# MasonMcGill/multipath-nn

Measured on AMD Instinct MI355X. Metric: images/sec training CIFAR-10 actor-net, higher is better.
Workload: dtype f32; 1 GPU; cifar10-ac: ac_chain(k_cpt=0) 8-block actor-routed chain, 32x32x3, 10 classes; global_batch=128, per_gpu_batch=128, parallelism=dp1, rccl_ranks=1, hip_graph=True, steps_per_graph=4, streams=1, clock_warmup_steps=96

## Files before the change

### multipath-nn_amd/csrc/lin.hip

```cpp
#include "common.h"
#include <cstddef>

struct LinFwdG {
    ActG a;  int HW;
    gptr<const float> w[2];  gptr<const float> b[2];  gptr<float> y[2];  int M[2];
    gptr<const float> k_cpt;  float alpha_cpt;  int extra_col[2];
    int n;
    gptr<float> kpart;  gptr<int> kcnt;
};
struct LinBwdG {
    ActG a;  int HW;
    gptr<const float> w[2];  gptr<const float> dy[2];  int M[2];
    gptr<float> dw[2];  gptr<float> db[2];
    gptr<float> dx;
    gptr<const float> k_cpt;  float alpha_cpt;  int extra_col[2];
    int n;
    gptr<float> dz_out;  gptr<double> red_out;  int red_nslot;
    gptr<float> kpart;  gptr<int> kcnt;
    float act_alpha;  gptr<const float> act_w;
};
static_assert(sizeof(LinFwdG) == sizeof(mpnn_lin_fwd_args) && offsetof(LinFwdG, y) == offsetof(mpnn_lin_fwd_args, y) &&
              offsetof(LinFwdG, k_cpt) == offsetof(mpnn_lin_fwd_args, k_cpt) && offsetof(LinFwdG, kcnt) == offsetof(mpnn_lin_fwd_args, kcnt),
              "LinFwdG mirrors mpnn_lin_fwd_args");
static_assert(sizeof(LinBwdG) == sizeof(mpnn_lin_bwd_args) && offsetof(LinBwdG, dw) == offsetof(mpnn_lin_bwd_args, dw) &&
// ... 280 lines not shown
#pragma unroll
            for (int s = 0; s < 8; ++s)
#pragma unroll
                for (int pp = 0; pp < LB_GP; ++pp) dx[pp] = __builtin_amdgcn_mfma_f32_16x16x4f32(ady[pp][s], wv[s], dx[pp], 0, 0, 0);
#pragma unroll
            for (int pp = 0; pp < LB_GP; ++pp)
#pragma unroll
                for (int s = 0; s < 4; ++s) {
                    accW[0] = __builtin_amdgcn_mfma_f32_16x16x4f32(xa[pp][s], bdy[pp][0][s], accW[0], 0, 0, 0);
                    accW[1] = __builtin_amdgcn_mfma_f32_16x16x4f32(xa[pp][s], bdy[pp][1][s], accW[1], 0, 0, 0);
                }
            asm volatile("" : "+a"(accW[0]), "+a"(accW[1]));
            mfma_drain();
            if (act_on) {
                const float a2 = 2.f * a.act_alpha;
#pragma unroll
                for (int pp = 0; pp < LB_GP; ++pp)
#pragma unroll
                    for (int q = 0; q < 4; ++q) {
                        const int rr = LB_ROWS * (pg + pp) + 4 * g + q;
                        const bool ok = rr < nr && f < K;
                        const float w = a.act_w[ok ? R0 + rr : R0];
                        dx[pp][q] += ok ? a2 * w * xa[pp][q] : 0.f;
                    }
            }
#pragma unroll
            for (int pp = 0; pp < LB_GP; ++pp)
#pragma unroll
                for (int q = 0; q < 4; ++q) {
                    const int rr = LB_ROWS * (pg + pp) + 4 * g + q;
                    if (rr < nr && f < K) {
                        if (a.dx) a.dx[(size_t)(R0 + rr) * K + f] = dx[pp][q];
                        if (fuse_bn) {
                            const float dz = xa[pp][q] > 0.f ? dx[pp][q] : 0.f;
                            a.dz_out[(size_t)(R0 + rr) * K + f] = dz;
                            r1 += dz; r2 += dz * xh[pp][q];
                        }
                    }
                }
        }
    }
    trace_stamp(4);
    float dbt = 0.f;
    if (blockIdx.x == 0) {
        float *dbp = tr + 512;
        dbp[tid] = dbs;
        __syncthreads();
        if (tid < 32) {
#pragma unroll
            for (int rg = 0; rg < 8; ++rg) dbt += dbp[rg * 32 + tid];
        }
    }
    if constexpr (RS) {
        if (Z > 1) {
            __shared__ int ticket;
            const gptr<float> part0 = a.kpart + (size_t)blockIdx.x * gridDim.z * MPNN_LIN_RS_TILE;
            const gptr<float> mine = part0 + (size_t)zi * MPNN_LIN_RS_TILE;
#pragma unroll
            for (int set = 0; set < 2; ++set)
#pragma unroll
                for (int q = 0; q < 4; ++q)
                    __hip_atomic_store(mine + (wid * 16 + 4 * g + q) * 32 + set * 16 + li, accW[set][q], __ATOMIC_RELAXED, __HIP_MEMORY_SCOPE_SYSTEM);
            if (blockIdx.x == 0 && tid < 32) __hip_atomic_store(mine + 2048 + tid, dbt, __ATOMIC_RELAXED, __HIP_MEMORY_SCOPE_SYSTEM);
            asm volatile("s_waitcnt vmcnt(0)" ::: "memory");
            __builtin_amdgcn_fence(__ATOMIC_RELEASE, "workgroup");
            __syncthreads();
            if (tid == 0) ticket = __hip_atomic_fetch_add(a.kcnt + blockIdx.x, 1, __ATOMIC_RELAXED, __HIP_MEMORY_SCOPE_SYSTEM);
            __syncthreads();
            if (ticket != Z - 1) { trace_stamp(5); goto bn_sums; }
            {
                float pv[2][4][MPNN_LIN_RSPLIT];
#pragma unroll
                for (int set = 0; set < 2; ++set)
#pragma unroll
                    for (int q = 0; q < 4; ++q)
#pragma unroll
                        for (int z = 0; z < MPNN_LIN_RSPLIT; ++z)
                            pv[set][q][z] = __hip_atomic_load(part0 + (size_t)(z < Z ? z : 0) * MPNN_LIN_RS_TILE + (wid * 16 + 4 * g + q) * 32 + set * 16 + li,
                                                              __ATOMIC_RELAXED, __HIP_MEMORY_SCOPE_SYSTEM);
                float pd[MPNN_LIN_RSPLIT];
#pragma unroll
                for (int z = 0; z < MPNN_LIN_RSPLIT; ++z)
                    pd[z] = (blockIdx.x == 0 && tid < 32) ? __hip_atomic_load(part0 + (size_t)(z < Z ? z : 0) * MPNN_LIN_RS_TILE + 2048 + tid, __ATOMIC_RELAXED, __HIP_MEMORY_SCOPE_SYSTEM) : 0.f;
#pragma unroll
                for (int set = 0; set < 2; ++set)
#pragma unroll
                    for (int q = 0; q < 4; ++q) {
                        float v = 0.f;
#pragma unroll
                        for (int z = 0; z < MPNN_LIN_RSPLIT; ++z) v += z < Z ? pv[set][q][z] : 0.f;
                        accW[set][q] = v;
                    }
                dbt = 0.f;
#pragma unroll
                for (int z = 0; z < MPNN_LIN_RSPLIT; ++z) dbt += z < Z ? pd[z] : 0.f;
                if (tid == 0) __hip_atomic_store(a.kcnt + blockIdx.x, 0, __ATOMIC_RELAXED, __HIP_MEMORY_SCOPE_SYSTEM);
            }
        }
    }
#pragma unroll
    for (int set = 0; set < 2; ++set) {
        const gptr<const float> wp = set ? a.w[1] : a.w[0];
        const gptr<float> dwp = set ? a.dw[1] : a.dw[0];
        if (!wp || !dwp) continue;
        const int M = set ? a.M[1] : a.M[0];
        const int krows = (set ? a.extra_col[1] : a.extra_col[0]) ? K + 1 : K;
// ... 57 lines not shown
```

### multipath-nn_amd/csrc/route.hip

```cpp
#include "common.h"

#define MSK MPNN_MAX_SINKS

#define RT_THREADS 512
#define RT_WAVES (RT_THREADS / 64)

__device__ __forceinline__ int4 uniform4(int4 v) {
    return make_int4(__builtin_amdgcn_readfirstlane(v.x), __builtin_amdgcn_readfirstlane(v.y),
                     __builtin_amdgcn_readfirstlane(v.z), __builtin_amdgcn_readfirstlane(v.w));
}

template <class P, class T> __device__ __forceinline__ void st_part(P p, T v) { __hip_atomic_store(p, v, __ATOMIC_RELAXED, __HIP_MEMORY_SCOPE_SYSTEM); }
template <class P> __device__ __forceinline__ auto ld_part(P p) { return __hip_atomic_load(p, __ATOMIC_RELAXED, __HIP_MEMORY_SCOPE_SYSTEM); }

struct RouteG {
    int net_type;  int n_nodes, n_leaves, n_switches, max_sinks;
    int optimistic, use_cls_err, want_grad;
    gptr<const int> nodes;  gptr<const int> sw_children;  gptr<const float> node_ops;
    gptr<const float> hyp;
    gptr<const float> k_cpt_vec;
    gptr<const float> r;
    gptr<const float> c_err;  gptr<const float> d_cor;
    gptr<float> p_tr, p_ev;
    gptr<float> w_cerr;
    gptr<float> dr;
    gptr<float> node_stat;
    gptr<double> loss;
    int n;  int n_total;
    gptr<float> stat_part;  gptr<int> stat_ticket;
};
static_assert(sizeof(RouteG) == sizeof(mpnn_route_args) && offsetof(RouteG, nodes) == offsetof(mpnn_route_args, nodes) &&
              offsetof(RouteG, loss) == offsetof(mpnn_route_args, loss) && offsetof(RouteG, n_total) == offsetof(mpnn_route_args, n_total) &&
              offsetof(RouteG, stat_ticket) == offsetof(mpnn_route_args, stat_ticket), "RouteG mirrors mpnn_route_args");

template <int RB, class A>
__device__ __forceinline__ void route_body(const A &a, const int blk, const int nblk) {
    extern __shared__ __attribute__((aligned(16))) float lds[];
    const int n = a.n, NN = a.n_nodes, MS = a.max_sinks;
    const bool det_stat = a.node_stat && a.stat_part && nblk > 2;
    trace_stamp(0); trace_note(6, 14);
    float *P = lds;
    float *PE = P + NN * RB;
    float *V = PE + NN * RB;
    float *O = V + NN * RB;
    float *RIN = O + NN * RB;
    float *CE = RIN + a.n_switches * MS * RB;
    float *DC = CE + a.n_leaves * RB;
    float *SM = DC + a.n_leaves * RB;
    int *ARG = (int *)(SM + a.n_switches * MS * RB);
    int4 *REC = (int4 *)(ARG + a.n_switches * RB);
    float *OPS = (float *)(REC + NN + 1);
    int *SWN = (int *)(OPS + NN);
    const int s0 = blk * RB;
// ... 247 lines not shown
    if (a.loss) {
        const double e = wave_sum_d(live ? (double)l_err : 0.0), c = wave_sum_d(live ? (double)l_cpt : 0.0);
        const double x = wave_sum_d(live ? (double)l_aux : 0.0), cnt = wave_sum_d((live && wave == 0) ? 1.0 : 0.0);
        double *lsum = (double *)lds;
        __syncthreads();
        if (lane_t == 0) { lsum[wave * 4] = e; lsum[wave * 4 + 1] = c; lsum[wave * 4 + 2] = x; lsum[wave * 4 + 3] = wave == 0 ? cnt : 0.0; }
        __syncthreads();
        if (threadIdx.x < 4) {
            double t = 0.0;
#pragma unroll
            for (int w = 0; w < RT_WAVES; ++w) t += lsum[w * 4 + threadIdx.x];
            if (det_stat) st_part(pcast<double>(a.stat_part + (size_t)nblk * NN * 2) + blk * 4 + threadIdx.x, t);
            else atomic_add_g(a.loss + threadIdx.x, t);
        }
    }
    if (det_stat) {
        int *last_s = (int *)lds + 128;
        asm volatile("s_waitcnt vmcnt(0)" ::: "memory");
        __syncthreads();
        if (threadIdx.x == 0) {
            __threadfence();
            *last_s = atomic_add_g(a.stat_ticket, 1) == nblk - 1;
        }
        __syncthreads();
        if (*last_s) {
            __threadfence();
            for (int i = threadIdx.x; i < 2 * NN; i += RT_THREADS) {
                float t = 0.f;
                for (int b = 0; b < nblk; ++b) t += ld_part(a.stat_part + (size_t)b * NN * 2 + i);
                a.node_stat[i] += t;
            }
            if (a.loss && threadIdx.x < 4) {
                const auto lp = pcast<const double>(a.stat_part + (size_t)nblk * NN * 2);
                double t = 0.0;
                for (int b = 0; b < nblk; ++b) t += ld_part(lp + b * 4 + threadIdx.x);
                a.loss[threadIdx.x] += t;
            }
            if (threadIdx.x == 0) *a.stat_ticket = 0;
        }
    }
    trace_stamp(5);
}

template <int RB>
__global__ __launch_bounds__(RT_THREADS) void route_k(const mpnn_route_args a) { route_body<RB>(a, blockIdx.x, gridDim.x); }

template <int RB>
__global__ __launch_bounds__(RT_THREADS) void route_multi_k(const mpnn_route_args *__restrict__ tab, const int wpn) {
    const int net = blockIdx.x / wpn;
    const RouteG a = ((const RouteG *)tab)[net];
    route_body<RB>(a, blockIdx.x - net * wpn, wpn);
}

int mpnn_trace_install_route(void *buf) { return mpnn_trace_install(buf); }

extern "C" int mpnn_route(const mpnn_route_args *args, void *stream) {
    if (!args || !args->nodes || !args->p_tr || !args->p_ev || (args->stat_part && !args->stat_ticket)) return MPNN_E_ARG;
    if (args->n_nodes > MPNN_MAX_NODES || args->max_sinks > MPNN_MAX_SINKS) return MPNN_E_SHAPE;
    if (args->n <= 0) return 0;
    const size_t per = (size_t)(4 * args->n_nodes + 2 * args->n_switches * args->max_sinks + args->n_switches + 2 * args->n_leaves) * 4;
    const size_t fix = (size_t)(args->n_nodes * 5 + 8 + args->n_switches) * 4;
    const size_t cap = 160 * 1024;
    const hipStream_t st = (hipStream_t)stream;
    const int n = args->n;
    static bool raised = false;
    if (!raised) {
        hipFuncSetAttribute((const void *)route_k<64>, hipFuncAttributeMaxDynamicSharedMemorySize, (int)cap);
        hipFuncSetAttribute((const void *)route_k<32>, hipFuncAttributeMaxDynamicSharedMemorySize, (int)cap);
        hipFuncSetAttribute((const void *)route_k<16>, hipFuncAttributeMaxDynamicSharedMemorySize, (int)cap);
        raised = true;
    }
    if (per * 64 + fix <= cap)      hipLaunchKernelGGL(route_k<64>, dim3((n + 63) / 64), dim3(RT_THREADS), per * 64 + fix, st, *args);
    else if (per * 32 + fix <= cap) hipLaunchKernelGGL(route_k<32>, dim3((n + 31) / 32), dim3(RT_THREADS), per * 32 + fix, st, *args);
    else if (per * 16 + fix <= cap) hipLaunchKernelGGL(route_k<16>, dim3((n + 15) / 16), dim3(RT_THREADS), per * 16 + fix, st, *args);
    else return MPNN_E_SHAPE;
    MPNN_LAUNCH_CHECK();
    return 0;
}

extern "C" int mpnn_route_multi(const mpnn_route_args *host_table, const mpnn_route_args *dev_table, int count, void *stream) {
    if (count <= 0) return 0;
    if (!host_table || !dev_table) return MPNN_E_ARG;
    const mpnn_route_args *args = host_table;
    for (int k = 0; k < count; ++k) {
        const mpnn_route_args &b = host_table[k];
        if (!b.nodes || !b.p_tr || !b.p_ev || (b.stat_part && !b.stat_ticket)) return MPNN_E_ARG;
        if (b.n != args->n || b.n_nodes != args->n_nodes || b.n_switches != args->n_switches || b.n_leaves != args->n_leaves ||
            b.max_sinks != args->max_sinks) return MPNN_E_ARG;
    }
    if (args->n_nodes > MPNN_MAX_NODES || args->max_sinks > MPNN_MAX_SINKS) return MPNN_E_SHAPE;
    if (args->n <= 0) return 0;
    const size_t per = (size_t)(4 * args->n_nodes + 2 * args->n_switches * args->max_sinks + args->n_switches + 2 * args->n_leaves) * 4;
    const size_t fix = (size_t)(args->n_nodes * 5 + 8 + args->n_switches) * 4;
    const size_t cap = 160 * 1024;
    const hipStream_t st = (hipStream_t)stream;
    const int n = args->n;
    static bool raised = false;
    if (!raised) {
        hipFuncSetAttribute((const void *)route_multi_k<64>, hipFuncAttributeMaxDynamicSharedMemorySize, (int)cap);
        hipFuncSetAttribute((const void *)route_multi_k<32>, hipFuncAttributeMaxDynamicSharedMemorySize, (int)cap);
        hipFuncSetAttribute((const void *)route_multi_k<16>, hipFuncAttributeMaxDynamicSharedMemorySize, (int)cap);
        raised = true;
    }
    if (per * 64 + fix <= cap)      { const int w = (n + 63) / 64; hipLaunchKernelGGL(route_multi_k<64>, dim3(w * count), dim3(RT_THREADS), per * 64 + fix, st, dev_table, w); }
    else if (per * 32 + fix <= cap) { const int w = (n + 31) / 32; hipLaunchKernelGGL(route_multi_k<32>, dim3(w * count), dim3(RT_THREADS), per * 32 + fix, st, dev_table, w); }
    else if (per * 16 + fix <= cap) { const int w = (n + 15) / 16; hipLaunchKernelGGL(route_multi_k<16>, dim3(w * count), dim3(RT_THREADS), per * 16 + fix, st, dev_table, w); }
    else return MPNN_E_SHAPE;
    MPNN_LAUNCH_CHECK();
    return 0;
}
```

### multipath-nn_amd/lib/_eng_planner.py

```python
import ctypes as C
import functools
import os

import numpy as np
import torch

from lib import _hip
from lib._eng_common import Launch, _attr, head_activity, head_parts


class Planner:

    def _wsplit(self, b, i, n, fused=False):
        H = b.H[i]
        tiles = n * (H // 16) * (H // 4) if H >= 16 else (n if H == 8 else (n + 3) // 4)
        nch = (b.Cin[i] + 15) // 16 + ((b.C[i - 1] + 15) // 16 if i > 0 else 0)
        groups = max(1, b.C[i] // 64) if b.C[i] % 64 == 0 else (b.C[i] // 32 if b.C[i] % 32 == 0 else b.C[i] // 16)
        if fused:
            groups = b.C[i] // 64 if b.C[i] % 64 == 0 else b.C[i] // 16
        budget = 512
        if fused:
            has_dgrad = 1 if (b.in_map is not None or i > 0) else 0
            dg_items = tiles * ((b.parent.C[b.in_map[i]] // 16 if b.parent is not None else 0) + (b.C[i - 1] // 16 if i > 0 else 0))
            slots = self.lib.mpnn_msconv_bwd_scale_slots(b.H[i], b.W[i], b.C[i], has_dgrad, 1 if i > 0 else 0, dg_items)
# ... 128 lines not shown
            return None
        used = sum(g * body[2] for g, body in zip(gx, bodies))
        while True:
            cand = [q for q in range(len(gx)) if gx[q] < bodies[q][3] and used + bodies[q][2] <= slots]
            if not cand:
                break
            q = max(cand, key=lambda q: -(-bodies[q][3] // gx[q]) * bodies[q][4])
            gx[q] += 1
            used += bodies[q][2]
        if os.environ.get('MPNN_PLAN_DEBUG'):
            print('level budget: %d slots, chain %.1f; ' % (slots, cands[lo]) + '; '.join(
                'm%d %s rows %d tiles %d -> gx %d (%d wgs, %d items/wg)' % (k, kind, rows, tiles, g, g * rows, -(-tiles // g))
                for (k, kind, rows, tiles, lat), g in zip(bodies, gx)))
        out = [dict(gxh=0, gxv=0, split=1) for _ in grp]
        for (k, kind, rows, tiles, lat), g in zip(bodies, gx):
            if self.co_share == 1:
                g = self._xcd_round(g)
            if kind == 'w':
                kb, b, i = grp[k]
                g = max(1, min(g, max(1, (12 << 20) // self._w_bytes(b, i))))
            out[k]['gxh' if kind == 'h' else 'gxv' if kind == 'v' else 'split'] = int(g)
        return out


    def program(self, mode, n, routed=False, gate=frozenset(), points=0):
        try:
            return self._program(mode, n, routed, frozenset(gate), int(points))
        finally:
            self.lib.mpnn_set_reserved_cus(0)


    def routed_prefix(self, n):
        table = self._ROUTED_PREFIX_GEN if self.generic_convs else self._ROUTED_PREFIX
        for lim, d0 in table:
            if n >= lim:
                return d0
        return table[-1][1]

    _ROUTED_PREFIX = ((6144, 1), (3072, 2), (1536, 3), (640, 4), (0, 6))
    _ROUTED_PREFIX_GEN = ((0, 1),)


    def _program(self, mode, n, routed, gate=frozenset(), points=0):
        if routed == 'auto':
            routed = n >= (self.routed_min_batch_gen if self.generic_convs else self.routed_min_batch)
        explicit = routed if (isinstance(routed, int) and not isinstance(routed, bool) and routed >= 1) else None
        routed = bool(routed) and mode != 'tr' and bool(self.switches) and self.net._net_kind != 'sr'
        if routed:
            routed = explicit if explicit is not None else self.routed_prefix(n)
        if mode == 'tr' and self.allreduce is not None and self.multi_stream:
            raise NotImplementedError('data-parallel training runs on the single-stream schedule (MPNN_STREAMS=0)')
        dp = mode == 'tr' and self.allreduce is not None
        reserve = self.dp_reserve_cus if (dp and len(self.dp_buckets) > 1) else 0
        key = (mode, n, self.multi_stream, self.group_fwd, routed, dp, self.bwd_levels, self.fold_clear, reserve, self.fuse_opt, self.co_share, gate) + \
            ((points,) if mode == 'ev+c' else ())
        if key in self._progs:
            return self._progs[key]
        self._ensure_capacity(n, mode == 'tr')
        if mode != 'tr':
            prog = self._progs[key] = self._program_ev(n, routed) if mode == 'ev' else self._program_cv(n, points) if mode == 'ev+c' else \
                self._program_pr(n, routed, mode == 'pr+p', gate)
            return prog
        if self.multi_stream and self.generic_convs:
            raise NotImplementedError('the multi-stream schedule has no launches for the general conv kernels (filters other '
                                      'than 3x3, maps other than the tuned squares): such nets run on the single-stream '
                                      'schedule (MPNN_STREAMS=0)')
        if self.multi_stream and any(len(b.children) > 1 for b in self.blocks):
            raise NotImplementedError('the multi-stream schedule serialises nothing between sibling blocks that '
                                      'accumulate into one gradient map: tree nets run on the single-stream schedule')
        prog = self._progs[key] = self._program_tr(n, dp, reserve)
        return prog


    def _program_tr(self, n, dp, reserve):
        sizes = sorted({h for b in self.blocks for h in b.H}, reverse=True)
        sid = {h: (0 if h == sizes[-1] else 1 + k) for k, h in enumerate(sizes)}
        self.n_streams = len(sizes) + 2
        fwd = self._label_map_launches(n) + self._lln_launches(n) + [Launch(None, 'fork')]
        if self.group_fwd and not self.multi_stream and self._groupable() and \
                all(b.parent is not None or b.in_map is None for b in self.blocks):
            for members in self._wavefront(self.blocks):
                fwd += self._conv_fwd_launches(members, n, 'tr')
        else:
            F = lambda b, i: 'F%d_%d' % (self.blocks.index(b), i)
            for b in self.blocks:
                for i in range(b.L):
                    fwd.append(self._conv_fwd_single(b, i, n, 'tr', None, 'msconv_fwd', stream=sid[b.H[i]],
                                                     waits=[F(b, i - 1)] if i > 0 else [], records=F(b, i)))
        fwd.append(Launch(None, 'join'))
        exit_fwd, bwd, fold = self._exit_launches(n)
        fwd += exit_fwd + [self._route_launch(n, 'tr', self.loss)]
        if dp and 'exit' in self.dp_buckets:
            bwd.append(Launch(None, 'bucket', tag='exit'))
        self.lib.mpnn_set_reserved_cus(reserve)
        convs, fused_opt = self._bwd_launches(n, sid, dp, reserve, fold)
        bwd += convs
        if dp:
            bwd.append(Launch(None, 'bucket', tag='end'))
        return dict(fwd=fwd, bwd=bwd, n=n, mode='tr', fold=fold, fused_opt=fused_opt)


    def _conv_fwd_args(self, b, i, n, mode, rows=None):
        train = mode == 'tr'
        a = _hip.ConvFwdArgs()
        a.a = self._act_of_input(b, i, n, _hip.ACT_BN_BATCH if train else _hip.ACT_BN_MOVING, fwd=train)
        cp = b.conv.params
        if i > 0:
            a.v, a.Cv = b.sp[i - 1].data_ptr(), b.C[i - 1]
            a.wv_pack = getattr(cp, 'w_vert_%i' % (i - 1)).data.data_ptr() if self.generic_convs else \
                self.packs[b.pack['w_vert_%i' % (i - 1)][0]:].data_ptr()
        if i < b.L - 1:
            a.pool_out = b.sp[i].data_ptr()
        a.wa_pack = getattr(cp, 'w_horz_%i' % i).data.data_ptr() if self.generic_convs else \
            self.packs[b.pack['w_horz_%i' % i][0]:].data_ptr()
        a.bias = getattr(b.conv.params, 'b_%i' % i).data.data_ptr()
        a.out = b.s[i].data_ptr()
        a.out_sum = self.dsum[b.sum_off[i]:].data_ptr() if train else None
        a.out_nslot = self._nslot(b, i)
        a.n, a.H, a.W, a.Cout = n, b.H[i], b.W[i], b.C[i]
        if rows is not None:
            a.idx, a.cnt = rows[0].data_ptr(), rows[1].data_ptr()
        return a


    @staticmethod
    def _conv_flops(b, i, n):
        (kh, kw), (kvh, kvw) = b.kh[i], b.kv[i] or (0, 0)
        return 2.0 * n * b.H[i] * b.W[i] * b.C[i] * (kh * kw * b.Cin[i] + (kvh * kvw * b.C[i - 1] if i > 0 else 0))


    def _conv_fwd_single(self, b, i, n, mode, rows, what, **kw):
        a = self._conv_fwd_args(b, i, n, mode, rows)
        self._keep.append(a)
        fl, tag = self._conv_flops(b, i, n), self._conv_tag(b, i)
        if self.generic_convs:
            return Launch(self._gen_fn('fwd'), what, C.byref(a), *b.kh[i], *(b.kv[i] or (0, 0)), flops=fl, tag=tag, **kw)
        return Launch(self.lib.mpnn_msconv_fwd, what, C.byref(a), flops=fl, tag=tag, **kw)


    @staticmethod
    def _conv_tag(b, i):
        hw = 'h%d' % b.H[i] if b.H[i] == b.W[i] else 'h%dx%d' % (b.H[i], b.W[i])
        return '%s %d+%d->%d' % (hw, b.Cin[i], b.C[i - 1] if i > 0 else 0, b.C[i])


    def _wavefront(self, blocks):
        depth = self._depths()
        kidx = {h: k for k, h in enumerate(sorted({h for b in self.blocks for h in b.H}, reverse=True))}
        levels = {}
        for b in blocks:
            for i in range(b.L):
                levels.setdefault(depth[id(b)] + kidx[b.H[i]], []).append((b, i))
        return [levels[d] for d in sorted(levels)]


    def _conv_fwd_launches(self, members, n, mode, rows=lambda b: None):
        lib, out = self.lib, []
        if not self._groupable():
            return [self._conv_fwd_single(b, i, n, mode, rows(b), 'fwd') for b, i in members]
        for c0 in range(0, len(members), 4):
            grp = members[c0:c0 + 4]
            arr = (_hip.ConvFwdArgs * len(grp))(*[self._conv_fwd_args(b, i, n, mode, rows(b)) for b, i in grp])
            dev_arr = _hip.to_device_table(list(arr), self.dev)
            self._keep += [arr, dev_arr]
            fl, tag = sum(self._conv_flops(b, i, n) for b, i in grp), ' | '.join(self._conv_tag(b, i) for b, i in grp)
            if self.co_share > 1:
                out.append(Launch(lib.mpnn_msconv_fwd_group_rep, 'fwd_group', arr, dev_arr.data_ptr(), len(grp), 1, self.co_share,
                                  flops=fl, tag=tag, host=arr))
            else:
                out.append(Launch(lib.mpnn_msconv_fwd_group, 'fwd_group', arr, dev_arr.data_ptr(), len(grp), flops=fl, tag=tag, host=arr))
        return out


    def _depths(self):
        depth = {}
        for b in self.blocks:
            depth[id(b)] = 0 if b.parent is None else depth[id(b.parent)] + 1
        return depth


    def _groupable(self):
        return not self.generic_convs and \
            all(c % 16 == 0 and not (c % 64 == 0 and h >= 16) for b in self.blocks for c, h in zip(b.C, b.H))


    def _exit_launches(self, n):
        lib, keep = self.lib, self._keep
        act_mode = _hip.ACT_BN_BATCH
        ϕ = self.net.hypers
        dyn = bool(getattr(ϕ, 'dyn_k_cpt', False))
        lin_f, lin_b, tail_f, tail_b = [], [], [], []
        MS = self.max_sinks
        kmax = 0
        for b in self.blocks:
            if not b.has_exit:
                continue
            L1 = b.L - 1
            K = b.H[L1] * b.W[L1] * b.C[L1]
            kmax = max(kmax, K)
            lf, lb = _hip.LinFwdArgs(), _hip.LinBwdArgs()
            tf, tb = _hip.ExitTailArgs(), _hip.ExitTailBwdArgs()
            a_in = _hip.act(b.s[L1], b.C[L1], act_mode, 0, self._bn(b, L1), n * b.H[L1] * b.W[L1])
            lf.a, lb.a = a_in, a_in
            lf.HW = lb.HW = b.H[L1] * b.W[L1]
            lf.n = lb.n = tf.n = n
            lf.k_cpt = lb.k_cpt = self.k_cpt.data_ptr()
            lf.alpha_cpt = lb.alpha_cpt = float(_attr(ϕ, 'α_cpt', 0.0))
            if K >= 512 and n <= 512:
                rg = (n + 15) // 16
                kpart = torch.empty(rg * _hip.LIN_KSLICES * 512, device=self.dev)
                kcnt = torch.zeros(rg, dtype=torch.int32, device=self.dev)
                keep += [kpart, kcnt]
                lf.kpart, lf.kcnt = kpart.data_ptr(), kcnt.data_ptr()
            if n <= 512:
                nblk = (K + 1 + 63) // 64
                bpart = torch.empty(nblk * _hip.LIN_RSPLIT * _hip.LIN_RS_TILE, device=self.dev)
                bcnt = torch.zeros(nblk, dtype=torch.int32, device=self.dev)
                keep += [bpart, bcnt]
                lb.kpart, lb.kcnt = bpart.data_ptr(), bcnt.data_ptr()
            lb.dx = b.dx.data_ptr()
            if not b.children and not self.multi_stream and not self.generic_exits:
                lb.dx = None
                lb.dz_out = b.dzg[L1].data_ptr()
                lb.red_out = self.dred[b.sum_off[L1]:].data_ptr()
                lb.red_nslot = self._nslot(b, L1)
            tf.mode = act_mode
            if b.head is not None:
                lt, _, tf.loss, tf.eps_ce = head_parts(b.head.layer)
                lf.w[0], lf.b[0], lf.y[0], lf.M[0] = lt.params.w.data.data_ptr(), lt.params.b.data.data_ptr(), b.z.data_ptr(), b.n_out
                lb.w[0], lb.dy[0], lb.M[0] = lf.w[0], b.dzh.data_ptr(), b.n_out
                lb.dw[0], lb.db[0] = lt.params.w.grad.data_ptr(), lt.params.b.grad.data_ptr()
                leaf = b.head.leaf_id
                tf.z, tf.y, tf.n_cls = b.z.data_ptr(), self._labels_of(b).data_ptr(), b.n_out
                tf.c_err = self.c_err[leaf * n:].data_ptr()
                tf.d_cor = self.d_cor[leaf * n:].data_ptr()
                tb.w_cerr = self.w_cerr[leaf * n:].data_ptr()
                tb.dz = b.dzh.data_ptr()
                lb.act_alpha, tb.act_z, tb.act_p = head_activity(b.head.layer)
                if lb.act_alpha:
                    lb.act_w = tb.w_cerr
            if b.router is not None:
                rc = b.router.comps
                l1, bn1, l2, bn2, l3 = rc[1], rc[2], rc[4], rc[5], rc[7]
                R, S = b.R, len(b.node.layer.sinks)
                sw = b.node.switch_id
                lf.w[1], lf.b[1], lf.y[1], lf.M[1] = l1.params.w.data.data_ptr(), l1.params.b.data.data_ptr(), b.h1.data_ptr(), R
                lb.w[1], lb.dy[1], lb.M[1] = lf.w[1], b.dh1.data_ptr(), R
                lb.dw[1], lb.db[1] = l1.params.w.grad.data_ptr(), l1.params.b.grad.data_ptr()
                lf.extra_col[1] = lb.extra_col[1] = 1 if dyn else 0
                tf.h1, tf.R, tf.n_sinks, tf.R2 = b.h1.data_ptr(), R, S, b.R2
                tf.g1, tf.b1 = bn1.params.γ.data.data_ptr(), bn1.params.β.data.data_ptr()
                tf.m1, tf.v1 = bn1.params.m_avg.data.data_ptr(), bn1.params.v_avg.data.data_ptr()
                tf.w2, tf.bias2 = l2.params.w.data.data_ptr(), l2.params.b.data.data_ptr()
                tf.g2, tf.b2 = bn2.params.γ.data.data_ptr(), bn2.params.β.data.data_ptr()
                tf.m2, tf.v2 = bn2.params.m_avg.data.data_ptr(), bn2.params.v_avg.data.data_ptr()
                tf.w3, tf.bias3 = l3.params.w.data.data_ptr(), l3.params.b.data.data_ptr()
                tf.h2 = b.h2.data_ptr()
                tf.r, tf.r_stride = self.r[sw * n * MS:].data_ptr(), MS
                tf.bn_save = b.bn_save.data_ptr()
                tf.bn_eps, tf.bn_decay = float(bn1.hypers.ϵ), float(bn1.hypers.d)
                tf.bn_eps2, tf.bn_decay2 = float(bn2.hypers.ϵ), float(bn2.hypers.d)
                tb.dr = self.dr[sw * n * MS:].data_ptr()
                tb.dh1 = b.dh1.data_ptr()
                if getattr(b, 'dh2', None) is not None:
                    tb.dh2 = b.dh2.data_ptr()
                tb.dg1, tb.db1 = bn1.params.γ.grad.data_ptr(), bn1.params.β.grad.data_ptr()
                tb.dw2, tb.dbias2 = l2.params.w.grad.data_ptr(), l2.params.b.grad.data_ptr()
                tb.dg2, tb.db2 = bn2.params.γ.grad.data_ptr(), bn2.params.β.grad.data_ptr()
                tb.dw3, tb.dbias3 = l3.params.w.grad.data_ptr(), l3.params.b.grad.data_ptr()
            tb.f = tf
            lin_f.append(lf); lin_b.append(lb); tail_f.append(tf); tail_b.append(tb)
        n_exit = len(lin_f)
        fold = n_exit > 0 and self.fold_clear
        if not n_exit:
            return [], [], fold
        if fold:
            tail_f[0].clear_f, tail_f[0].n_clear_f = self.node_stat.data_ptr(), self.node_stat.numel()
            tail_f[0].clear_d, tail_f[0].n_clear_d = self.loss.data_ptr(), self.loss.numel()
        t_lf, t_lb = _hip.to_device_table(lin_f, self.dev), _hip.to_device_table(lin_b, self.dev)
        t_tf, t_tb = _hip.to_device_table(tail_f, self.dev), _hip.to_device_table(tail_b, self.dev)
        keep += [t_lf, t_lb, t_tf, t_tb]
        if self.generic_exits:
            lin_fwd = Launch(lib.mpnn_lin_fwd_gen, 'lin_fwd', t_lf.data_ptr(), n_exit, n, host=lin_f)
        elif n <= 512:
            lin_fwd = Launch(lib.mpnn_lin_fwd_ks, 'lin_fwd', t_lf.data_ptr(), n_exit, n, kmax, host=lin_f)
        else:
            lin_fwd = Launch(lib.mpnn_lin_fwd, 'lin_fwd', t_lf.data_ptr(), n_exit, n, host=lin_f)
        gen_tails = self.generic_exits or n > 128
        lin_bwd = lib.mpnn_lin_bwd_gen if self.generic_exits else lib.mpnn_lin_bwd_rs if n <= 512 else lib.mpnn_lin_bwd
        fwd = [lin_fwd, Launch(lib.mpnn_exit_tail_fwd_gen if gen_tails else lib.mpnn_exit_tail_fwd, 'exit_tail_fwd',
                               t_tf.data_ptr(), n_exit, n, host=tail_f)]
        bwd = [Launch(lib.mpnn_exit_tail_bwd_gen if gen_tails else lib.mpnn_exit_tail_bwd, 'exit_tail_bwd', t_tb.data_ptr(), n_exit, n,
                      host=tail_b),
               Launch(lin_bwd, 'lin_bwd', t_lb.data_ptr(), n_exit, n, kmax, host=lin_b)]
        return fwd, bwd, fold


    def _route_launch(self, n, mode, loss):
        ϕ, kind = self.net.hypers, self.net._net_kind
        ra = _hip.RouteArgs()
        ra.net_type = {'sr': _hip.NET_SR, 'actor': _hip.NET_ACTOR, 'critic': _hip.NET_CRITIC}[kind]
        ra.n_nodes, ra.n_leaves, ra.n_switches, ra.max_sinks = len(self.nodes), len(self.leaves), len(self.switches), self.max_sinks
        ra.optimistic = int(bool(getattr(ϕ, 'optimistic', False)))
        ra.use_cls_err = int(bool(getattr(ϕ, 'use_cls_err', False)))
        ra.want_grad = 1 if mode == 'tr' else 0
        ra.nodes, ra.sw_children, ra.node_ops = self.node_tab.data_ptr(), self.kid_tab.data_ptr(), self.node_ops.data_ptr()
        ra.hyp = self.hyp.data_ptr()
        ra.k_cpt_vec = self.k_cpt.data_ptr() if bool(getattr(ϕ, 'dyn_k_cpt', False)) else None
        ra.r, ra.c_err, ra.d_cor = self.r.data_ptr(), self.c_err.data_ptr(), self.d_cor.data_ptr()
        ra.p_tr, ra.p_ev, ra.w_cerr, ra.dr = self.p_tr.data_ptr(), self.p_ev.data_ptr(), self.w_cerr.data_ptr(), self.dr.data_ptr()
        ra.node_stat = self.node_stat.data_ptr() if mode == 'tr' else None
        if mode == 'tr':
            need = (n + 15) // 16 * (len(self.nodes) * 2 + 8)
            if self._stat_part is None or self._stat_part.numel() < need:
                self._stat_part = torch.zeros(need, device=self.dev)
                self._stat_ticket = torch.zeros(4, dtype=torch.int32, device=self.dev)
            ra.stat_part, ra.stat_ticket = self._stat_part.data_ptr(), self._stat_ticket.data_ptr()
            self._keep += [self._stat_part, self._stat_ticket]
        ra.loss = loss.data_ptr()
        ra.n, ra.n_total = n, n
        self._keep.append(ra)
        return Launch(self.lib.mpnn_route, 'route', C.byref(ra), host=ra)


    def _bwd_launches(self, n, sid, dp, reserve, fold):
        lib, keep = self.lib, self._keep
        call = functools.partial(Launch, reserve=reserve)
        Gn = lambda b, i: 'G%d_%d' % (self.blocks.index(b), i)
        bwd = [Launch(None, 'fork')]
        dz_written = set()
        slab_size = 0
        slab_members = []
        slab_params = set()
        levels = []
        cut_kb = self.dp_cut_block if dp else None

        def make_block(kb, b):
            cp = b.conv.params
            L1 = b.L - 1
            pre = []
            if not b.children and (self.multi_stream or not b.has_exit or self.generic_exits):
                ctx = self._bn_ctx(b, L1, n, with_red=False)
                pre.append(call(lib.mpnn_bn_bwd_reduce, 'bn_bwd_reduce', b.dx.data_ptr(), C.byref(ctx),
                                b.dzg[L1].data_ptr(), self.dred[b.sum_off[L1]:].data_ptr(),
                                n * b.H[L1] * b.W[L1], stream=sid[b.H[L1]]))
            g_ctx = None
            if self.multi_stream or self.generic_convs:
                ctx = self._bn_ctx(b, L1, n)
                pre.append(call(lib.mpnn_bn_bwd_apply, 'bn_bwd_apply', b.dzg[L1].data_ptr(), C.byref(ctx),
                                n * b.H[L1] * b.W[L1], stream=sid[b.H[L1]], records=Gn(b, L1)))
            else:
                g_ctx = C.pointer(self._bn_ctx(b, L1, n))

            def vert_args(i):
                a = _hip.DgradVertArgs()
                fine = self._bn_ctx(b, i - 1, n)
                a.g, a.Cg = b.dzg[i].data_ptr(), b.C[i]
                if i == L1 and g_ctx is not None:
                    a.g_ctx = g_ctx
                a.w_pack = getattr(cp, 'w_vert_%i' % (i - 1)).data.data_ptr() if self.generic_convs else \
                    self.packs[b.pack['w_vert_%i' % (i - 1)][1]:].data_ptr()
                a.fine = C.pointer(fine)
                a.fine_has_dz = 1 if b.has_dz[i - 1] else 0
                a.dz_g_fine = b.dzg[i - 1].data_ptr()
                a.n, a.H, a.W, a.Cout = n, b.H[i], b.W[i], b.C[i - 1]
                keep.append(a)
                return a

            def horz_args(i):
                pb, j = b.parent, b.in_map[i]
                a = _hip.DgradHorzArgs()
                a.g, a.Cg = b.dzg[i].data_ptr(), b.C[i]
                if i == L1 and g_ctx is not None:
                    a.g_ctx = g_ctx
                a.w_pack = getattr(cp, 'w_horz_%i' % i).data.data_ptr() if self.generic_convs else \
                    self.packs[b.pack['w_horz_%i' % i][1]:].data_ptr()
                first = (id(pb), j) not in dz_written
                dz_written.add((id(pb), j))
# ... 84 lines not shown
                    (kb, b, i), _ = grp[0]
                    h, v, w = built[0][:3]
                    kv = b.kv[i] or (0, 0)
                    if h is not None:
                        bwd.append(call(self._gen_fn('dgrad_horz'), 'dgrad_horz', C.byref(h), *b.kh[i], flops=fl_h(b, i), tag=tag))
                    if v is not None:
                        bwd.append(call(self._gen_fn('dgrad_vert'), 'dgrad_vert', C.byref(v), *kv, flops=fl_v(b, i), tag=tag))
                    bwd.append(call(self._gen_fn('wgrad'), 'wgrad', C.byref(w), *b.kh[i], *kv, flops=self._conv_flops(b, i, n),
                                    tag=tag))
                elif len(built) == 1 and built[0][3] is None:
                    h, v, w = built[0][:3]
                    bwd.append(call(lib.mpnn_msconv_bwd_scale, 'bwd_scale', C.byref(h) if h is not None else None,
                                    C.byref(v) if v is not None else None, C.byref(w), flops=fl, tag=tag))
                else:
                    mem = (_hip.BwdMember * len(built))()
                    for m, (h, v, w, bud, _, _) in zip(mem, built):
                        m.horz = C.pointer(h) if h is not None else None
                        m.vert = C.pointer(v) if v is not None else None
                        m.wgrad = C.pointer(w)
                        m.wg_horz, m.wg_vert = bud['gxh'], bud['gxv']
                    dev_rec = torch.empty(rec_bytes * len(built), dtype=torch.uint8, device=self.dev)
                    keep += [mem, dev_rec]
                    levels.append((mem, dev_rec))
                    if self.co_share > 1:
                        bwd.append(call(lib.mpnn_msconv_bwd_level_rep, 'bwd_scale', mem, len(built), 1, dev_rec.data_ptr(),
                                        flops=fl, tag=tag, host=mem))
                    else:
                        bwd.append(call(lib.mpnn_msconv_bwd_level, 'bwd_scale', mem, len(built), dev_rec.data_ptr(),
                                        flops=fl, tag=tag, host=mem))
                if last_cut is not None and g == last_cut:
                    if any(m[0] for m in slab_members):
                        mid = len(bwd)
                    bwd.append(Launch(None, 'bucket', tag='mid'))
        else:
            wg_streams = (len(sid), len(sid) + 1)
            for kb, b in enumerate(reversed(self.blocks)):
                pre, vert_args, horz_args, wgrad_args = make_block(kb, b)
                bwd += pre
                L1 = b.L - 1
                for i in range(L1, 0, -1):
                    bwd.append(call(lib.mpnn_msconv_dgrad_vert, 'dgrad_vert', C.byref(vert_args(i)), flops=fl_v(b, i),
                                    tag='h%d %d->%d' % (b.H[i], b.C[i], b.C[i - 1]),
                                    stream=sid[b.H[i - 1]], waits=[Gn(b, i)], records=Gn(b, i - 1)))
                if b.parent is not None:
                    for i in range(b.L):
                        bwd.append(call(lib.mpnn_msconv_dgrad_horz, 'dgrad_horz', C.byref(horz_args(i)), flops=fl_h(b, i),
                                        tag='h%d %d->%d' % (b.H[i], b.C[i], b.parent.C[b.in_map[i]]),
                                        stream=sid[b.H[i]]))
                for i in range(b.L):
                    bwd.append(call(lib.mpnn_msconv_wgrad, 'wgrad', C.byref(wgrad_args(i)), flops=self._conv_flops(b, i, n),
                                    tag=self._conv_tag(b, i), stream=wg_streams[i % 2], waits=[Gn(b, i)]))
        bwd.append(Launch(None, 'join'))

        keep_ptr = self.dsum_last.data_ptr() if fold else None
        fused_opt = False
        if slab_size:
            slab = torch.empty(slab_size, device=self.dev)
            rows, srows, first = [], [], 0
            for want_cut in (True, False):
                for is_cut, r, ptrs, sr in slab_members:
                    if is_cut == want_cut:
                        rows += r
                        srows += sr
                        for a, field, off in ptrs:
                            setattr(a, field, slab[off:].data_ptr())
                if want_cut:
                    first = len(rows) // 6
            tab = torch.tensor(rows, dtype=torch.int32, device=self.dev)
            keep += [slab, tab]
            n_items = len(rows) // 6
            if mid is not None:
                bwd.insert(mid, call(lib.mpnn_slab_reduce, 'slab_reduce', slab.data_ptr(), self.G.data_ptr(), tab.data_ptr(), first))
            fused_opt = not dp and self.fuse_opt and not self.multi_stream
            if fused_opt:
                bwd.append(self._finish_opt_launch(n, slab, tab, n_items, srows, slab_params, keep_ptr))
            else:
                bwd.append(call(lib.mpnn_backward_finish, 'backward_finish', slab.data_ptr(), self.G.data_ptr(),
                                tab[6 * first:].data_ptr(), n_items - first, self.dsum.data_ptr(), self.dred.data_ptr(),
                                self.S.data_ptr(), self.bn_table.data_ptr(), self.n_bn, self.bn_decay, n, keep_ptr))
        else:
            bwd.append(call(lib.mpnn_bn_finalize, 'bn_finalize', self.dsum.data_ptr(), self.dred.data_ptr(),
                            self.S.data_ptr(), self.G.data_ptr(), self.bn_table.data_ptr(), self.n_bn,
                            self.bn_decay, n, keep_ptr))
        self._upload_level_records(levels)
        return bwd, fused_opt


    def _finish_opt_launch(self, n, slab, tab, n_items, srows, slab_params, keep_ptr):
        bn_opt, fused_bn = [], set()
        for b in self.blocks:
            for i in range(b.L):
                bn = b.bns[i].params
                bn_opt += [b.node.idx, int(np.float32(bn.γ.l2).view(np.int32)), int(np.float32(bn.β.l2).view(np.int32)), 0]
                fused_bn |= {id(bn.γ), id(bn.β)}
        segs = self.seg_host.reshape(-1, _hip.SEG_INTS)
        plain = [segs[k] for k, pid in enumerate(self._seg_owner) if pid not in slab_params and pid not in fused_bn]
        t_seg = torch.tensor(srows, dtype=torch.int32, device=self.dev)
        t_bno = torch.tensor(bn_opt, dtype=torch.int32, device=self.dev)
        t_plain = torch.from_numpy(np.concatenate(plain) if plain else np.zeros(_hip.SEG_INTS, np.int32)).to(self.dev)
        self._keep += [t_seg, t_bno, t_plain]
        talr = 1 if (self.net._net_kind != 'sr' and getattr(self.net.hypers, 'talr', False)) else 0
        fin = _hip.FinishNet()
        fin.slabs, fin.slab_table, fin.n_items, fin.item_seg = slab.data_ptr(), tab.data_ptr(), n_items, t_seg.data_ptr()
        fin.sums, fin.reds, fin.state = self.dsum.data_ptr(), self.dred.data_ptr(), self.S.data_ptr()
        fin.bn_table, fin.n_bn, fin.bn_opt, fin.n_img, fin.sums_keep = self.bn_table.data_ptr(), self.n_bn, t_bno.data_ptr(), n, keep_ptr
        fin.params, fin.accum, fin.grads = self.P.data_ptr(), self.A.data_ptr(), self.G.data_ptr()
        fin.node_stat, fin.hyp, fin.talr, fin.inv_n, fin.grad_scale = self.node_stat.data_ptr(), self.hyp.data_ptr(), talr, 1.0 / n, 1.0
        fin.w_eq, fin.packs = (self.w_eq.data_ptr() if self.w_eq is not None else None), self.packs.data_ptr()
        fin.plain_seg, fin.n_plain = t_plain.data_ptr(), len(plain)
        f = [getattr(fin, name) for name, _ in fin._fields_]
        return Launch(self.lib.mpnn_backward_finish_opt, 'backward_finish', *f[:10], self.bn_decay, *f[10:], host=fin)


    def _upload_level_records(self, levels):
        for mem, dev_rec in levels:
            host = (C.c_char * dev_rec.numel())()
            if self.co_share > 1:
                _hip.check(self.lib.mpnn_msconv_bwd_level_prepare_rep(mem, len(mem), 1, C.cast(host, C.c_void_p)), 'bwd_level records')
            else:
                _hip.check(self.lib.mpnn_msconv_bwd_level_prepare(mem, len(mem), C.cast(host, C.c_void_p)), 'bwd_level records')
            dev_rec.copy_(torch.frombuffer(bytearray(host.raw), dtype=torch.uint8))
```

### multipath-nn_amd/lib/_hip.py

```python
import ctypes as C
import os

_HERE = os.path.dirname(os.path.abspath(__file__))
LIB_PATH = os.environ.get('MPNN_HIP_LIB') or os.path.join(os.path.dirname(_HERE), 'libmpnn_hip.so')

ACT_IDENTITY, ACT_BN_BATCH, ACT_BN_MOVING, ACT_RELU = 0, 1, 2, 3
NET_SR, NET_ACTOR, NET_CRITIC = 0, 1, 2
LOSS_CE, LOSS_SQ, LOSS_SQ_LIN = 0, 1, 2
HYP_LR, HYP_MU, HYP_TAU, HYP_EPS, HYP_KCPT, HYP_KDEC, HYP_KCRE, HYP_ARTR, HYP_N = 0, 1, 2, 3, 4, 5, 6, 7, 16
MAX_NODES, MAX_SINKS = 128, 4
BN_SLOTS = 16
SEG_INTS = 12
SLAB_ITEM = 1024
LIN_KSLICES = 8
LIN_RSPLIT = 8
LIN_RS_TILE = 2080


def slab_item_size(n_split):
    size = SLAB_ITEM
    while size > 64 and (256 // (size // 4)) * 16 < n_split:
        size //= 2
    return size

P = C.c_void_p


class Act(C.Structure):
    _fields_ = [('x', P), ('sum', P), ('gamma', P), ('beta', P), ('m_avg', P), ('v_avg', P),
                ('eps', C.c_float), ('cnt', C.c_int), ('C', C.c_int), ('shift', C.c_int), ('mode', C.c_int),
                ('nslot', C.c_int)]


class ConvFwdArgs(C.Structure):
    _fields_ = [('a', Act), ('v', P), ('Cv', C.c_int), ('wa_pack', P), ('wv_pack', P), ('bias', P),
                ('out', P), ('pool_out', P), ('out_sum', P), ('out_nslot', C.c_int), ('n', C.c_int), ('H', C.c_int), ('W', C.c_int),
                ('Cout', C.c_int), ('idx', P), ('cnt', P)]


class BnCtx(C.Structure):
    _fields_ = [('s', P), ('bn', Act), ('red', P), ('red_nslot', C.c_int)]


class DgradHorzArgs(C.Structure):
    _fields_ = [('g', P), ('Cg', C.c_int), ('g_ctx', C.POINTER(BnCtx)), ('w_pack', P), ('dy_extra', P),
                ('prev', C.POINTER(BnCtx)),
                ('out', P), ('red_out', P), ('n', C.c_int), ('H', C.c_int), ('W', C.c_int), ('Cout', C.c_int),
                ('accumulate', C.c_int)]


class DgradVertArgs(C.Structure):
    _fields_ = [('g', P), ('Cg', C.c_int), ('g_ctx', C.POINTER(BnCtx)), ('w_pack', P), ('fine', C.POINTER(BnCtx)),
                ('fine_has_dz', C.c_int),
                ('dz_g_fine', P), ('n', C.c_int), ('H', C.c_int), ('W', C.c_int), ('Cout', C.c_int)]


class WgradArgs(C.Structure):
    _fields_ = [('a', Act), ('v', P), ('Cv', C.c_int), ('g', P), ('g_ctx', C.POINTER(BnCtx)), ('dwa', P), ('dwv', P),
                ('db', P),
                ('split_stride', C.c_long), ('n', C.c_int), ('H', C.c_int), ('W', C.c_int), ('Cout', C.c_int), ('n_split', C.c_int)]


BWD_LEVEL_MAX = 4


class BwdMember(C.Structure):
    _fields_ = [('horz', C.POINTER(DgradHorzArgs)), ('vert', C.POINTER(DgradVertArgs)), ('wgrad', C.POINTER(WgradArgs)),
                ('wg_horz', C.c_int), ('wg_vert', C.c_int)]


class LinFwdArgs(C.Structure):
    _fields_ = [('a', Act), ('HW', C.c_int), ('w', P * 2), ('b', P * 2), ('y', P * 2), ('M', C.c_int * 2),
                ('k_cpt', P), ('alpha_cpt', C.c_float), ('extra_col', C.c_int * 2), ('n', C.c_int),
                ('kpart', P), ('kcnt', P)]


# ... 286 lines not shown
```

### multipath-nn_amd/lib/_plan.py

```python
import os

import torch

from lib import _hip
from lib._eng_common import (BLOCK_COMPS, CAPTURE_MODE, HEAD_COMPS, OPT_CHUNK, ROUTER_COMPS, BoundInput, _attr, _Block, _kind, _nf,
                             _Node)
from lib._eng_structure import Structure
from lib._eng_alloc import Allocation
from lib._eng_planner import Planner
from lib._eng_eval import EvalPrograms
from lib._eng_run import Runner
from lib._eng_dp import DataParallelSections
from lib._eng_ksteps import KStepGraphs
from lib._eng_inspect import Inspection
from lib._eng_stream import StreamedPredict


class Engine(Structure, Allocation, Planner, EvalPrograms, Runner, StreamedPredict, DataParallelSections, KStepGraphs, Inspection):
    def __init__(self, net, device=None, n_max=128):
        self.net = net
        self.lib = _hip.load()
        if not torch.cuda.is_available():
            raise _hip.HipError('no GPU visible: the multipath-nn hot path runs on MI355X only')
        if device is None:
            device = 'cuda:%d' % int(os.environ.get('LOCAL_RANK', '0'))
        self.dev = torch.device(device)
        torch.cuda.set_device(self.dev)
        self.n_max = self.n_max_bwd = 0
        self.use_graph = bool(int(os.environ.get('MPNN_GRAPH', '1')))
        self.multi_stream = bool(int(os.environ.get('MPNN_STREAMS', '0')))
        self.group_fwd = bool(int(os.environ.get('MPNN_FWD_GROUP', '1')))
        self.bwd_levels = bool(int(os.environ.get('MPNN_BWD_LEVELS', '1')))
        self.routed_min_batch = 512
        self.routed_min_batch_gen = 512
        self.fold_clear = bool(int(os.environ.get('MPNN_FOLD_CLEAR', '1')))
        self._acc_clean = False
        self._streams = []
        self._event_keep = []
        self.n_streams = 1
        self.world = 1
        self.allreduce = None
        self.allreduce_capturable = False
        self.dp_agree = None
        self.dp_quiesce = None
        self.dp_one_graph = bool(int(os.environ.get('MPNN_DP_ONE_GRAPH', '1')))
        self.dp_reserve_cus = int(os.environ.get('MPNN_DP_RESERVE_CUS', '0'))
        self.dp_bucket_opt = bool(int(os.environ.get('MPNN_DP_BUCKET_OPT', '0')))
        self._opt_stream = None
        self.prologue = None
        self.prologue_slot = None
        self.fuse_opt = bool(int(os.environ.get('MPNN_FUSE_OPT', '1')))
        self.co_share = 1
        self._keep = []
        self._init_stream_state()
        self._init_kstep_state()
        self._progs = {}
        self._graphs = {}
        self._gen = 0
        self._hyp_epoch = 0
        self._reserved = 0
        self._last_fold = False
        self._stat_part = self._stat_ticket = None
        self._views_key = None
        self._sums_cache = None
        self._draw_bufs = {}
        self._classify()
        self._layout()
        self._alloc_params()
        self.init_params(net.hypers.__dict__.get('seed'))
        self._ensure_capacity(n_max)
        self.last_n = 0
        self.last_mode = 'ev'
```

Baseline: 277,200 images/s.

## Route exit linear-backward split-K partials into the fused slab reduce instead of ticket reduction

```diff
diff --git a/multipath-nn_amd/csrc/lin.hip b/multipath-nn_amd/csrc/lin.hip
--- a/multipath-nn_amd/csrc/lin.hip
+++ b/multipath-nn_amd/csrc/lin.hip
@@ -356,6 +356,33 @@
         }
     }
     if constexpr (RS) {
+        if (!a.kcnt && a.kpart) {
+            const gptr<const float> w0 = a.w[0], w1 = a.w[1];
+            const int e0 = a.extra_col[0] ? 1 : 0, e1 = a.extra_col[1] ? 1 : 0;
+            const int S0 = w0 ? (K + e0) * a.M[0] : 0, S1 = w1 ? (K + e1) * a.M[1] : 0;
+            const int B0 = w0 ? a.M[0] : 0, B1 = w1 ? a.M[1] : 0;
+            const int o_dw1 = (S0 + 3) & ~3, o_db0 = o_dw1 + ((S1 + 3) & ~3), o_db1 = o_db0 + ((B0 + 3) & ~3), stride = o_db1 + ((B1 + 3) & ~3);
+            const gptr<float> mine = a.kpart + (size_t)zi * stride;
+#pragma unroll
+            for (int set = 0; set < 2; ++set) {
+                if (!(set ? w1 : w0)) continue;
+                const int M = set ? a.M[1] : a.M[0];
+                const int krows = K + (set ? e1 : e0);
+                const gptr<float> dwp = mine + (set ? o_dw1 : 0);
+                if (li < M) {
+#pragma unroll
+                    for (int q = 0; q < 4; ++q) {
+                        const int fr = k0 + wid * 16 + 4 * g + q;
+                        if (fr < krows) dwp[(size_t)fr * M + li] = accW[set][q];
+                    }
+                }
+            }
+            if (blockIdx.x == 0 && tid < 32) {
+                const int s = tid >> 4, m = tid & 15;
+                if ((s ? w1 : w0) && m < (s ? B1 : B0)) mine[(s ? o_db1 : o_db0) + m] = dbt;
+            }
+            goto bn_sums;
+        }
         if (Z > 1) {
             __shared__ int ticket;
             const gptr<float> part0 = a.kpart + (size_t)blockIdx.x * gridDim.z * MPNN_LIN_RS_TILE;
diff --git a/multipath-nn_amd/csrc/route.hip b/multipath-nn_amd/csrc/route.hip
--- a/multipath-nn_amd/csrc/route.hip
+++ b/multipath-nn_amd/csrc/route.hip
@@ -1,4 +1,5 @@
 #include "common.h"
+#include <initializer_list>
 
 #define MSK MPNN_MAX_SINKS
 
@@ -352,6 +353,15 @@
     route_body<RB>(a, blockIdx.x - net * wpn, wpn);
 }
 
+static bool route_raise_lds(const void *k64, const void *k32, const void *k16, int cap) {
+    for (const void *k : {k64, k32, k16})
+        if (hipFuncSetAttribute(k, hipFuncAttributeMaxDynamicSharedMemorySize, cap) != hipSuccess) {
+            (void)hipGetLastError();
+            return false;
+        }
+    return true;
+}
+
 int mpnn_trace_install_route(void *buf) { return mpnn_trace_install(buf); }
 
 extern "C" int mpnn_route(const mpnn_route_args *args, void *stream) {
@@ -365,9 +375,7 @@
     const int n = args->n;
     static bool raised = false;
     if (!raised) {
-        hipFuncSetAttribute((const void *)route_k<64>, hipFuncAttributeMaxDynamicSharedMemorySize, (int)cap);
-        hipFuncSetAttribute((const void *)route_k<32>, hipFuncAttributeMaxDynamicSharedMemorySize, (int)cap);
-        hipFuncSetAttribute((const void *)route_k<16>, hipFuncAttributeMaxDynamicSharedMemorySize, (int)cap);
+        if (!route_raise_lds((const void *)route_k<64>, (const void *)route_k<32>, (const void *)route_k<16>, (int)cap)) return MPNN_E_SHAPE;
         raised = true;
     }
     if (per * 64 + fix <= cap)      hipLaunchKernelGGL(route_k<64>, dim3((n + 63) / 64), dim3(RT_THREADS), per * 64 + fix, st, *args);
@@ -397,9 +405,8 @@
     const int n = args->n;
     static bool raised = false;
     if (!raised) {
-        hipFuncSetAttribute((const void *)route_multi_k<64>, hipFuncAttributeMaxDynamicSharedMemorySize, (int)cap);
-        hipFuncSetAttribute((const void *)route_multi_k<32>, hipFuncAttributeMaxDynamicSharedMemorySize, (int)cap);
-        hipFuncSetAttribute((const void *)route_multi_k<16>, hipFuncAttributeMaxDynamicSharedMemorySize, (int)cap);
+        if (!route_raise_lds((const void *)route_multi_k<64>, (const void *)route_multi_k<32>, (const void *)route_multi_k<16>, (int)cap))
+            return MPNN_E_SHAPE;
         raised = true;
     }
     if (per * 64 + fix <= cap)      { const int w = (n + 63) / 64; hipLaunchKernelGGL(route_multi_k<64>, dim3(w * count), dim3(RT_THREADS), per * 64 + fix, st, dev_table, w); }
diff --git a/multipath-nn_amd/lib/_eng_planner.py b/multipath-nn_amd/lib/_eng_planner.py
--- a/multipath-nn_amd/lib/_eng_planner.py
+++ b/multipath-nn_amd/lib/_eng_planner.py
@@ -204,7 +204,8 @@
             raise NotImplementedError('data-parallel training runs on the single-stream schedule (MPNN_STREAMS=0)')
         dp = mode == 'tr' and self.allreduce is not None
         reserve = self.dp_reserve_cus if (dp and len(self.dp_buckets) > 1) else 0
-        key = (mode, n, self.multi_stream, self.group_fwd, routed, dp, self.bwd_levels, self.fold_clear, reserve, self.fuse_opt, self.co_share, gate) + \
+        key = (mode, n, self.multi_stream, self.group_fwd, routed, dp, self.bwd_levels, self.fold_clear, reserve, self.fuse_opt, self.co_share, gate,
+               self.exit_split_sum) + \
             ((points,) if mode == 'ev+c' else ())
         if key in self._progs:
             return self._progs[key]
@@ -240,12 +241,14 @@
                     fwd.append(self._conv_fwd_single(b, i, n, 'tr', None, 'msconv_fwd', stream=sid[b.H[i]],
                                                      waits=[F(b, i - 1)] if i > 0 else [], records=F(b, i)))
         fwd.append(Launch(None, 'join'))
-        exit_fwd, bwd, fold = self._exit_launches(n)
+        split_sum = self.exit_split_sum and not self.generic_exits and n <= 512 and _hip.lin_rs_groups(n, n) == 2 and \
+            not (dp and 'exit' in self.dp_buckets)
+        exit_fwd, bwd, fold, exit_split = self._exit_launches(n, split_sum)
         fwd += exit_fwd + [self._route_launch(n, 'tr', self.loss)]
         if dp and 'exit' in self.dp_buckets:
             bwd.append(Launch(None, 'bucket', tag='exit'))
         self.lib.mpnn_set_reserved_cus(reserve)
-        convs, fused_opt = self._bwd_launches(n, sid, dp, reserve, fold)
+        convs, fused_opt = self._bwd_launches(n, sid, dp, reserve, fold, exit_split)
         bwd += convs
         if dp:
             bwd.append(Launch(None, 'bucket', tag='end'))
@@ -336,12 +339,13 @@
             all(c % 16 == 0 and not (c % 64 == 0 and h >= 16) for b in self.blocks for c, h in zip(b.C, b.H))
 
 
-    def _exit_launches(self, n):
+    def _exit_launches(self, n, split_sum=False):
         lib, keep = self.lib, self._keep
         act_mode = _hip.ACT_BN_BATCH
         ϕ = self.net.hypers
         dyn = bool(getattr(ϕ, 'dyn_k_cpt', False))
         lin_f, lin_b, tail_f, tail_b = [], [], [], []
+        split_members = []
         MS = self.max_sinks
         kmax = 0
         for b in self.blocks:
@@ -364,7 +368,7 @@
                 kcnt = torch.zeros(rg, dtype=torch.int32, device=self.dev)
                 keep += [kpart, kcnt]
                 lf.kpart, lf.kcnt = kpart.data_ptr(), kcnt.data_ptr()
-            if n <= 512:
+            if n <= 512 and not split_sum:
                 nblk = (K + 1 + 63) // 64
                 bpart = torch.empty(nblk * _hip.LIN_RSPLIT * _hip.LIN_RS_TILE, device=self.dev)
                 bcnt = torch.zeros(nblk, dtype=torch.int32, device=self.dev)
@@ -420,12 +424,21 @@
                 tb.dw2, tb.dbias2 = l2.params.w.grad.data_ptr(), l2.params.b.grad.data_ptr()
                 tb.dg2, tb.db2 = bn2.params.γ.grad.data_ptr(), bn2.params.β.grad.data_ptr()
                 tb.dw3, tb.dbias3 = l3.params.w.grad.data_ptr(), l3.params.b.grad.data_ptr()
+            if split_sum:
+                has = (b.head is not None, b.router is not None)
+                offs, stride = _hip.lin_rs_part_layout(K, (lb.M[0], lb.M[1]), (lb.extra_col[0], lb.extra_col[1]), has)
+                prms = ([head_parts(b.head.layer)[0].params] if has[0] else [None]) + ([b.router.comps[1].params] if has[1] else [None])
+                tensors = [(q.w, offs[s]) for s, q in enumerate(prms) if q is not None] + \
+                    [(q.b, offs[2 + s]) for s, q in enumerate(prms) if q is not None]
+                assert all(q is None or (q.w.size == (K + (1 if lb.extra_col[s] else 0)) * lb.M[s] and q.b.size == lb.M[s])
+                           for s, q in enumerate(prms))
+                split_members.append((lb, stride, tensors))
             tb.f = tf
             lin_f.append(lf); lin_b.append(lb); tail_f.append(tf); tail_b.append(tb)
         n_exit = len(lin_f)
         fold = n_exit > 0 and self.fold_clear
         if not n_exit:
-            return [], [], fold
+            return [], [], fold, None
         if fold:
             tail_f[0].clear_f, tail_f[0].n_clear_f = self.node_stat.data_ptr(), self.node_stat.numel()
             tail_f[0].clear_d, tail_f[0].n_clear_d = self.loss.data_ptr(), self.loss.numel()
@@ -445,7 +458,7 @@
         bwd = [Launch(lib.mpnn_exit_tail_bwd_gen if gen_tails else lib.mpnn_exit_tail_bwd, 'exit_tail_bwd', t_tb.data_ptr(), n_exit, n,
                       host=tail_b),
                Launch(lin_bwd, 'lin_bwd', t_lb.data_ptr(), n_exit, n, kmax, host=lin_b)]
-        return fwd, bwd, fold
+        return fwd, bwd, fold, (lin_b, t_lb, split_members) if split_sum else None
 
 
     def _route_launch(self, n, mode, loss):
@@ -475,7 +488,7 @@
         return Launch(self.lib.mpnn_route, 'route', C.byref(ra), host=ra)
 
 
-    def _bwd_launches(self, n, sid, dp, reserve, fold):
+    def _bwd_launches(self, n, sid, dp, reserve, fold, exit_split=None):
         lib, keep = self.lib, self._keep
         call = functools.partial(Launch, reserve=reserve)
         Gn = lambda b, i: 'G%d_%d' % (self.blocks.index(b), i)
@@ -666,6 +679,23 @@
                                     tag=self._conv_tag(b, i), stream=wg_streams[i % 2], waits=[Gn(b, i)]))
         bwd.append(Launch(None, 'join'))
 
+        if exit_split is not None:
+            Z = _hip.lin_rs_groups(n, n)
+            item = _hip.slab_item_size(Z)
+            for lb, stride, tensors in exit_split[2]:
+                off = slab_size
+                slab_size += Z * stride
+                rows, srows = [], []
+                for prm, o in tensors:
+                    l2b, eqo, pk = self._opt_info[id(prm)]
+                    for k in range(0, prm.size, item):
+                        cnt = min(item, prm.size - k)
+                        rows += [off + o + k, prm.offset + k, cnt, Z, stride, 0]
+                        srows += [prm.offset + k, cnt, prm.node, prm.is_router, l2b, eqo + k if eqo >= 0 else -1,
+                                  pk[0], pk[1], pk[2], pk[3], pk[4], 0]
+                    slab_params.add(id(prm))
+                slab_members.append((False, rows, [(lb, 'kpart', off)], srows))
+
         keep_ptr = self.dsum_last.data_ptr() if fold else None
         fused_opt = False
         if slab_size:
@@ -682,6 +712,8 @@
                     first = len(rows) // 6
             tab = torch.tensor(rows, dtype=torch.int32, device=self.dev)
             keep += [slab, tab]
+            if exit_split is not None:
+                exit_split[1].copy_(_hip.to_device_table(exit_split[0], self.dev))
             n_items = len(rows) // 6
             if mid is not None:
                 bwd.insert(mid, call(lib.mpnn_slab_reduce, 'slab_reduce', slab.data_ptr(), self.G.data_ptr(), tab.data_ptr(), first))
diff --git a/multipath-nn_amd/lib/_hip.py b/multipath-nn_amd/lib/_hip.py
--- a/multipath-nn_amd/lib/_hip.py
+++ b/multipath-nn_amd/lib/_hip.py
@@ -22,6 +22,23 @@
     while size > 64 and (256 // (size // 4)) * 16 < n_split:
         size //= 2
     return size
+
+def lin_rs_groups(n, n_max):
+    g = max(1, min(LIN_RSPLIT, (n_max + 63) // 64))
+    p = (n + 15) // 16
+    ppw = (p + g - 1) // g
+    return (p + ppw - 1) // ppw if ppw else 0
+
+
+def lin_rs_part_layout(K, M, extra_col, present):
+    r4 = lambda x: (x + 3) // 4 * 4
+    S = [(K + (1 if extra_col[s] else 0)) * M[s] if present[s] else 0 for s in (0, 1)]
+    B = [M[s] if present[s] else 0 for s in (0, 1)]
+    o_dw1 = r4(S[0])
+    o_db0 = o_dw1 + r4(S[1])
+    o_db1 = o_db0 + r4(B[0])
+    return (0, o_dw1, o_db0, o_db1), o_db1 + r4(B[1])
+
 
 P = C.c_void_p
 
diff --git a/multipath-nn_amd/lib/_plan.py b/multipath-nn_amd/lib/_plan.py
--- a/multipath-nn_amd/lib/_plan.py
+++ b/multipath-nn_amd/lib/_plan.py
@@ -50,6 +50,7 @@
         self.prologue = None
         self.prologue_slot = None
         self.fuse_opt = bool(int(os.environ.get('MPNN_FUSE_OPT', '1')))
+        self.exit_split_sum = bool(int(os.environ.get('MPNN_EXIT_SPLIT_SUM', '1')))
         self.co_share = 1
         self._keep = []
         self._init_stream_state()
```

After: 276,700 images/s. No clear change (-0.2%).
